# effree/EM-Spec

Hardware: AMD Instinct MI355X
Metric: reassigned spectrogram columns/sec (4096-pt, hop 256, 48 kHz) (higher is better)
Workload: dtype f32

## Files before the change

### em-spec_amd/csrc/emspec_api.cpp

```cpp
#include "emspec_engine.h"
#ifdef EMSPEC_DIAG
#pragma GCC visibility push(default)
#include "../../include/emspec_debug.h"
#pragma GCC visibility pop
#endif
#include <algorithm>
#include <cmath>
#include <cstdio>
#include <cstdlib>
#include <cstring>
#include <map>
#include <new>
#include <string>
#include <vector>

using namespace emspec;

namespace {
thread_local std::string g_create_error = "";
}

namespace emspec {
int fail(const emspec_engine* e, int code, const std::string& msg) {
    if (e) e->err = msg; else g_create_error = msg;
// ... 113 lines not shown
    p.h_tw.resize(n);
    const double pi = 3.14159265358979323846;
    for (int q = 0; q < n / 2; ++q) {
        const double a = 2.0 * pi * (double)q / (double)n;
        p.h_tw[2 * q] = (float)std::cos(a);
        p.h_tw[2 * q + 1] = (float)(-std::sin(a));
    }
    for (int q = 0; q < n / 4; ++q) {
        p.h_tw[2 * (q + n / 4)] = p.h_tw[2 * q + 1];
        p.h_tw[2 * (q + n / 4) + 1] = -p.h_tw[2 * q];
    }
    p.h_tw[2 * (n / 4)] = 0.0f;
    p.h_tw[2 * (n / 4) + 1] = -1.0f;
    const int R = e->cfg.rows;
    p.h_ebin.resize(R + 1);
    const double ratio = (double)e->cfg.fmax_hz / (double)e->cfg.fmin_hz;
    for (int r = 0; r <= R; ++r)
        p.h_ebin[r] = e->custom_edges_hz.empty()
                          ? (float)((double)e->cfg.fmin_hz * spec_pow(ratio, (double)r / (double)R) * (double)n /
                                    (double)e->cfg.sample_rate)
                          : (float)((double)e->custom_edges_hz[r] * (double)n / (double)e->cfg.sample_rate);
    for (int r = 0; r < R; ++r)
        if (!(p.h_ebin[r] < p.h_ebin[r + 1])) return fail(e, EMSPEC_ERR_INVALID_ARG, "row edges are not strictly increasing in float32 (too many rows for this range)");
    HIPCHK(e, hipMalloc(&p.d_tw, sizeof(float) * n));
    HIPCHK(e, hipMalloc(&p.d_ebin, sizeof(float) * (R + 1)));
    HIPCHK(e, hipMemcpy(p.d_tw, p.h_tw.data(), sizeof(float) * n, hipMemcpyHostToDevice));
    HIPCHK(e, hipMemcpy(p.d_ebin, p.h_ebin.data(), sizeof(float) * (R + 1), hipMemcpyHostToDevice));
    if (e->exact()) {
        std::vector<double> tw((size_t)n), eb((size_t)R + 1);
        for (int q = 0; q <= n / 8; ++q) {
            double c, sn;
            cos_sin_octant(2.0 * pi * (double)q / (double)n, &c, &sn);
            tw[2 * q] = c;
            tw[2 * q + 1] = -sn;
            if (q > 0) {
                tw[2 * (n / 4 - q)] = sn;
                tw[2 * (n / 4 - q) + 1] = -c;
            }
        }
        for (int q = 0; q < n / 4; ++q) {
            tw[2 * (q + n / 4)] = tw[2 * q + 1];
            tw[2 * (q + n / 4) + 1] = -tw[2 * q];
        }
        tw[2 * (n / 4)] = 0.0;
        tw[2 * (n / 4) + 1] = -1.0;
        for (int r = 0; r <= R; ++r)
// ... 9 lines not shown
        HIPCHK(e, hipMemcpy(p.d_tw64, tw.data(), sizeof(double) * n, hipMemcpyHostToDevice));
        HIPCHK(e, hipMemcpy(p.d_ebin64, eb.data(), sizeof(double) * (R + 1), hipMemcpyHostToDevice));
    }
    auto ins = e->plans.emplace(n, std::move(p));
    *out = &ins.first->second;
    return EMSPEC_OK;
}

int get_band_plan(emspec_engine* e, int n, int row0, int rows, Plan** out) {
    const auto key = std::make_tuple(n, row0, rows);
    auto it = e->band_plans.find(key);
    if (it != e->band_plans.end()) { *out = &it->second; return EMSPEC_OK; }
    Plan* full;
    int rc;
    if ((rc = get_plan(e, n, &full))) return rc;
    if (row0 < 0 || rows < 1 || row0 + rows > full->rows) return fail(e, EMSPEC_ERR_INVALID_ARG, "band outside the row table");
    Plan p;
    p.n = n;
    p.row0 = row0;
    p.rows = rows;
    p.d_tw = full->d_tw;
    p.d_tw64 = full->d_tw64;
    p.h_ebin.assign(full->h_ebin.begin() + row0, full->h_ebin.begin() + row0 + rows + 1);
    HIPCHK(e, hipMalloc(&p.d_ebin, sizeof(float) * (rows + 1)));
    HIPCHK(e, hipMemcpy(p.d_ebin, p.h_ebin.data(), sizeof(float) * (rows + 1), hipMemcpyHostToDevice));
    if (e->exact()) {
        HIPCHK(e, hipMalloc(&p.d_ebin64, sizeof(double) * (rows + 1)));
        HIPCHK(e, hipMemcpy(p.d_ebin64, full->d_ebin64 + row0, sizeof(double) * (rows + 1), hipMemcpyDeviceToDevice));
        HIPCHK(e, hipMemcpy(&p.h_e0, full->d_ebin64 + row0, sizeof(double), hipMemcpyDeviceToHost));
        HIPCHK(e, hipMemcpy(&p.h_eR, full->d_ebin64 + row0 + rows, sizeof(double), hipMemcpyDeviceToHost));
    }
    auto ins = e->band_plans.emplace(key, std::move(p));
    *out = &ins.first->second;
    return EMSPEC_OK;
}

PlanDev plan_dev(const emspec_engine* e, const Plan& p, int hop, int reassign) {
    PlanDev d;
    d.tw = p.d_tw;
    d.ebin = p.d_ebin;
    d.rows = p.rows;
    d.log_rows = e->custom_edges_hz.empty() ? 1 : 0;
    d.D = latency(p.n, hop, reassign);
    d.reassign = reassign ? 1 : 0;
    d.hop = hop;
    d.tscale = (float)((double)p.n / 2.0 / (double)hop);
    const double pk = (double)p.n / 4.0;
    d.pfloor_abs = (float)((double)e->cfg.power_floor * pk * pk);
    d.shared = comm_shares_device(e) ? 1 : 0;
    return d;
}

ExactPlanDev exact_plan_dev(const emspec_engine* e, const Plan& p, int hop, int reassign) {
    ExactPlanDev d;
    d.tw = p.d_tw64;
    d.ebin = p.d_ebin64;
    d.rows = p.rows;
    d.log_rows = e->custom_edges_hz.empty() ? 1 : 0;
    d.D = latency(p.n, hop, reassign);
    d.reassign = reassign ? 1 : 0;
    d.hop = hop;
    d.tscale = (double)p.n / 2.0 / (double)hop;
    const double pk = (double)p.n / 4.0;
    d.pfloor = (double)e->cfg.power_floor * pk * pk;
    int log2n = 0;
// ... 457 lines not shown


int emspec_debug_occupy(emspec_engine* e, int32_t groups, int32_t usec, void* hip_stream) {
    if (!e || groups < 1 || groups > 4096 || usec < 1 || usec > 2000000) return fail(e, EMSPEC_ERR_INVALID_ARG, "bad argument");
    HIPCHK(e, hipSetDevice(e->device));
    HIPCHK(e, launch_occupy(groups, usec, reinterpret_cast<unsigned*>(e->d_lut) + 256, (hipStream_t)hip_stream));
    return EMSPEC_OK;
}

int emspec_debug_row_lookup(emspec_engine* e, int32_t n, const float* kh, int64_t count, int32_t* out_hint,
                            int32_t* out_exact) {
    if (!e || !kh || !out_hint || !out_exact || count < 0) return fail(e, EMSPEC_ERR_INVALID_ARG, "null argument");
    int rc = check_shape(e, n, 1);
    if (rc) return rc;
    HIPCHK(e, hipSetDevice(e->device));
    Plan* p;
    if ((rc = get_plan(e, n, &p))) return rc;
    float* d_kh = nullptr; int32_t *d_a = nullptr, *d_b = nullptr;
    hipError_t r = hipMalloc(&d_kh, count * 4 + 4);
    if (r == hipSuccess) r = hipMalloc(&d_a, count * 4 + 4);
    if (r == hipSuccess) r = hipMalloc(&d_b, count * 4 + 4);
    if (r == hipSuccess) r = hipMemcpyAsync(d_kh, kh, count * 4, hipMemcpyHostToDevice, e->stream);
    if (r == hipSuccess) r = launch_row_lookup_probe(p->d_ebin, e->cfg.rows, d_kh, count, d_a, d_b, e->stream);
    if (r == hipSuccess) r = hipMemcpyAsync(out_hint, d_a, count * 4, hipMemcpyDeviceToHost, e->stream);
    if (r == hipSuccess) r = hipMemcpyAsync(out_exact, d_b, count * 4, hipMemcpyDeviceToHost, e->stream);
    if (r == hipSuccess) r = hipStreamSynchronize(e->stream);
    (void)hipFree(d_kh); (void)hipFree(d_a); (void)hipFree(d_b);
    HIPCHK(e, r);
    return EMSPEC_OK;
}

int emspec_debug_recip(emspec_engine* e, const float* d, int64_t count, float* out_short, float* out_ieee) {
    if (!e || !d || !out_short || !out_ieee || count < 0) return fail(e, EMSPEC_ERR_INVALID_ARG, "null argument");
    HIPCHK(e, hipSetDevice(e->device));
    float *d_in = nullptr, *d_a = nullptr, *d_b = nullptr;
    hipError_t r = hipMalloc(&d_in, count * 4 + 4);
    if (r == hipSuccess) r = hipMalloc(&d_a, count * 4 + 4);
    if (r == hipSuccess) r = hipMalloc(&d_b, count * 4 + 4);
    if (r == hipSuccess) r = hipMemcpyAsync(d_in, d, count * 4, hipMemcpyHostToDevice, e->stream);
    if (r == hipSuccess) r = launch_recip_probe(d_in, count, d_a, d_b, e->stream);
    if (r == hipSuccess) r = hipMemcpyAsync(out_short, d_a, count * 4, hipMemcpyDeviceToHost, e->stream);
    if (r == hipSuccess) r = hipMemcpyAsync(out_ieee, d_b, count * 4, hipMemcpyDeviceToHost, e->stream);
    if (r == hipSuccess) r = hipStreamSynchronize(e->stream);
    (void)hipFree(d_in); (void)hipFree(d_a); (void)hipFree(d_b);
    HIPCHK(e, r);
    return EMSPEC_OK;
// ... 267 lines not shown
```

### em-spec_amd/csrc/emspec_device.h

```cpp
#pragma once
#include <hip/hip_runtime.h>
#include <stdint.h>

namespace emspec {

struct PlanDev {
    const float2* tw;
    const float* ebin;
    int rows;
    int log_rows;
    int D;
    int reassign;
    int hop;
    float tscale;
    float pfloor_abs;
    int shared;
};

struct SegPlan { int seglen; int nlong; int tail; int short_last; };
__device__ __forceinline__ bool seg_of_block(const SegPlan& sp, int64_t C, int& s, int64_t& c0, int64_t& c1) {
    if (!sp.short_last) {
        s = (int)blockIdx.y;
        c0 = (int64_t)blockIdx.x * sp.seglen;
        c1 = (c0 + sp.seglen < C) ? c0 + sp.seglen : C;
// ... 150 lines not shown
        }
        int r0 = (int)((__log2f(kh) - l2e0) * rscale);
        r0 = max(0, min(r0, R - 1));
        const float lo = eb[r0], hi = eb[r0 + 1];
        r0 += (kh >= hi) ? 1 : 0;
        r0 -= (kh < lo) ? 1 : 0;
        return r0;
    }
    __device__ __forceinline__ int row_signed(float kh) const {
        if (wtop) return in_range(kh) ? row_unchecked(kh) : -1;
        return row_unchecked(kh);
    }
    __device__ __forceinline__ int row_signed_log(float kh) const {
        int r0 = (int)((__log2f(kh) - l2e0) * rscale);
        r0 = max(0, min(r0, R - 1));
        const float lo = eb[r0], hi = eb[r0 + 1];
        r0 += (kh >= hi) ? 1 : 0;
        r0 -= (kh < lo) ? 1 : 0;
        return r0;
    }
    __device__ __forceinline__ int operator()(float kh) const { return in_range(kh) ? row_unchecked(kh) : -1; }
};

constexpr float kPowerMax = 1.0e36f;
constexpr float kFastMinFloor = 1.0e-27f;

__device__ __forceinline__ float recip_normal(float d) {
    const float r = __builtin_amdgcn_rcpf(d);
    const float e = __builtin_fmaf(-d, r, 1.0f);
    const float r1 = __builtin_fmaf(e, r, r);
    const float rem = __builtin_fmaf(-d, r1, 1.0f);
    const float q1 = __builtin_fmaf(rem, r1, r1);
    const float rem2 = __builtin_fmaf(-d, q1, 1.0f);
    return __builtin_fmaf(rem2, r1, q1);
}

struct BinOut { float power; int dcol; int row; };

__device__ __forceinline__ float twice_minus(float c, float s) { return __builtin_fmaf(2.0f, c, -s); }

struct YT { float yr, yi, tr, ti; };
__device__ __forceinline__ YT split_yt(float2 z, float2 w) {
    YT o;
    o.yr = z.x + w.x; o.yi = z.y - w.y; o.tr = z.y + w.y; o.ti = w.x - z.x;
    return o;
}
// ... 33 lines not shown
    return o;
}

__device__ __forceinline__ BinOut reassign_core_fast(const PlanDev& pl, const HintLookup& lk, int k,
                                                     const YT& m, const YT& c, const YT& p) {
    const float Ar = twice_minus(c.yr, m.yr + p.yr), Ai = twice_minus(c.yi, m.yi + p.yi);
    const float Br = twice_minus(c.tr, m.tr + p.tr), Bi = twice_minus(c.ti, m.ti + p.ti);
    const float Dr = m.yr - p.yr, Di = m.yi - p.yi;
    const float den = __builtin_fmaf(Ar, Ar, Ai * Ai);
    BinOut o;
    o.power = den * 0.015625f;
    const float numT = __builtin_fmaf(Br, Ar, Bi * Ai);
    const float numF = __builtin_fmaf(Dr, Ar, Di * Ai);
    const float inv = recip_normal(den);
    const float cf = __builtin_floorf(__builtin_fmaf(numT * inv, pl.tscale, 0.5f));
    const bool ok = (o.power >= pl.pfloor_abs) && (o.power <= kPowerMax) && (__builtin_fabsf(cf) <= (float)pl.D);
    const int rr = lk.row_signed_log((float)k + numF * inv);
    o.dcol = ok ? (int)cf : 0;
    o.row = (ok && (unsigned)rr < (unsigned)lk.R) ? rr : -1;
    return o;
}
__device__ __host__ __forceinline__ bool emspec_plan_is_fast(const PlanDev& pl) {
    return pl.reassign && pl.log_rows && pl.pfloor_abs >= kFastMinFloor;
}

__device__ __forceinline__ BinOut reassign_bin(const PlanDev& pl, const float* eb, int wtop, int k,
                                               float2 zm, float2 z0, float2 zp,
                                               float2 wm, float2 w0, float2 wp) {
    ExactLookup lk{eb, pl.rows, wtop};
    return reassign_core(pl, lk, k, split_yt(zm, wm), split_yt(z0, w0), split_yt(zp, wp));
}

__device__ __forceinline__ unsigned lds_accumulate_counted(float* cell, float p, bool want) {
    unsigned* c = reinterpret_cast<unsigned*>(cell);
    bool todo = want;
    unsigned rounds = 0;
    while (__builtin_amdgcn_ballot_w64(todo) != 0ull) {
        ++rounds;
        if (todo) {
            const unsigned old = __hip_atomic_exchange(c, 0xFFFFFFFFu, __ATOMIC_RELAXED, __HIP_MEMORY_SCOPE_WORKGROUP);
            if (old != 0xFFFFFFFFu) {
                __hip_atomic_store(cell, __uint_as_float(old) + p, __ATOMIC_RELAXED, __HIP_MEMORY_SCOPE_WORKGROUP);
                todo = false;
            }
        }
    }
// ... 56 lines not shown
```

### em-spec_amd/csrc/emspec_engine.h

```cpp
#pragma once
#pragma GCC visibility push(default)
#include "../../include/emspec.h"
#pragma GCC visibility pop
#include "emspec_launch.h"

#include <functional>
#include <map>
#include <string>
#include <tuple>
#include <vector>

struct emspec_engine;
namespace emspec {
struct Plan {
    int n = 0;
    int row0 = 0, rows = 0;
    float2* d_tw = nullptr;
    float* d_ebin = nullptr;
    std::vector<float> h_tw, h_ebin;
    double2* d_tw64 = nullptr;
    double* d_ebin64 = nullptr;
    double h_e0 = 0.0, h_eR = 0.0;
};
struct LiveState {
    int S = 0, n = 0, hop = 0, reassign = -1, D = 0;
    int n_high = 0, split = 0, shift = 0, D_high = 0;
    int slots_high = 0;
    void* d_cells_high = nullptr; size_t cells_high_bytes = 0;
    int form = 0;
    int slots = 0;
    int mmax = 0;
    int64_t cap = 0;
    int ring_mask = 0;
    std::vector<int64_t> fed, emitted, seen, newbase;
    std::vector<int> pend;
    void* d_cells = nullptr; size_t cells_bytes = 0;
    float* d_sring = nullptr; size_t sring_bytes = 0;
    unsigned* d_done = nullptr; size_t done_bytes = 0;
    float* d_raw = nullptr; size_t raw_bytes = 0;
    float* d_pstate = nullptr; size_t pstate_bytes = 0;
    void* h_desc = nullptr; size_t desc_bytes = 0;
    float* h_fresh = nullptr; size_t fresh_bytes = 0;
// ... 92 lines not shown
```

### em-spec_amd/csrc/emspec_launch.h

```cpp
#pragma once
#include <hip/hip_runtime.h>
#include <stdint.h>
#include "emspec_device.h"

namespace emspec {

struct LiveStream {
    long long j0;
    long long newbase;
    int frames;
    int newcount;
    int out_at;
    int flush;
};
struct LiveSinks {
    const LiveStream* streams = nullptr;
    LiveStream uni{};
    int uniform = 0;
    const float* fresh = nullptr;
    long long fresh_stride = 0;
    float* sring = nullptr;
    int ring_mask = 0;
    unsigned* done = nullptr;
    float* out_db = nullptr;
// ... 86 lines not shown
hipError_t launch_live_post(const LiveSinks& lv, const float* raw, int raw_cols, int rows, int D, float sm, float agc, float db_top,
                            const DbMap& dm, float* pstate, int S, hipStream_t st);
int64_t wire_bound_bytes(int64_t columns, int rows);
int64_t wire_fixed_bytes(int64_t columns, int rows);
size_t wire_scratch_bytes(int64_t columns);
hipError_t launch_wire_pack(const uint8_t* index, int64_t columns, int rows, uint8_t* wire, void* scratch, hipStream_t st);
hipError_t launch_wire_unpack(const uint8_t* wire, int64_t columns, int rows, uint8_t* index, hipStream_t st);
hipError_t launch_reduce_columns(const float* db_in, const uint8_t* idx_in, int S, int64_t C, int R, int f, size_t in_stride,
                                 size_t out_stride, const uint8_t* lut, float* db_out, uint8_t* idx_out, uint8_t* rgba_out,
                                 hipStream_t st);
hipError_t launch_peaks(const float* db, int64_t columns, int R, int k, float min_db, void* peaks, hipStream_t st);
enum { kPcmS16 = 1, kPcmS24 = 2, kPcmS32 = 3, kPcmF32 = 4, kPcmMaxChannels = 8, kPcmMaxViews = 8 };
struct PcmMix { float w[kPcmMaxViews * kPcmMaxChannels]; };
hipError_t launch_pcm_decode(const void* src, int sample_type, int channels, int views, const float* mix, int sources, int64_t frames,
                             int64_t src_stride_bytes, float* out, int64_t out_stride, hipStream_t st);
bool fused_supported(int n, int hop, int rows, int reassign);
int device_cus();
#ifdef EMSPEC_DIAG
int fused_waves_per_group();
int fused_read_errflag();
hipError_t launch_row_lookup_probe(const float* ebin, int rows, const float* kh, int64_t count, int32_t* out_hint,
                                   int32_t* out_exact, hipStream_t st);
hipError_t launch_occupy(int groups, int usec, unsigned* sink, hipStream_t st);
hipError_t launch_recip_probe(const float* d, int64_t count, float* out_short, float* out_ieee, hipStream_t st);
hipError_t launch_recip64_probe(const double* d, int64_t count, double* out_short, double* out_ieee, hipStream_t st);
#endif

}
```

### em-spec_amd/csrc/fused.hip.inc

```
#include "fused_r8.hip.inc"
#include "fused_n8192.hip.inc"
#include "fused_small.hip.inc"
#include "fused_n16384.hip.inc"
#include "fused_pp.hip.inc"
#ifdef EMSPEC_DIAG
#include "diag/fused_r16.hip.inc"
#include "diag/fused_r8t.hip.inc"
#include "diag/fused_pp3.hip.inc"
#endif
namespace emspec {

#ifdef EMSPEC_DIAG
static int fused_variant() {
    static int v = -1;
    if (v < 0) {
        const char* e = getenv("EMSPEC_FUSED_VARIANT");
        v = 0;
        if (e && e[0] == 'r' && e[1] == '1') v = 1;
        if (e && e[0] == 'r' && e[1] == '8' && e[2] == 't') v = 2;
        if (e && e[0] == 'r' && e[1] == '8' && e[2] != 't') v = 3;
        if (e && e[0] == 'p' && e[1] == 'p' && e[2] == 't') v = 4;
        if (e && e[0] == 'p' && e[1] == 'p' && e[2] == '3') v = 5;
    }
    return v;
}
static int* fused_errflag() {
    static int* p[64] = {};
    int dev = 0;
    (void)hipGetDevice(&dev);
    if (!p[dev & 63]) {
        if (hipMalloc(&p[dev & 63], sizeof(int)) != hipSuccess) return nullptr;
        (void)hipMemset(p[dev & 63], 0, sizeof(int));
    }
    return p[dev & 63];
}
int fused_read_errflag() {
    int v = 0;
    int* p = fused_errflag();
    if (p) (void)hipMemcpy(&v, p, sizeof(int), hipMemcpyDeviceToHost);
    return v;
}
int fused_waves_per_group() { return fused_variant() == 1 ? 8 : 16; }
static bool diag_no_fused() {
    static int off = -1;
    if (off < 0) { const char* e = getenv("EMSPEC_NO_FUSED"); off = (e && e[0] == '1') ? 1 : 0; }
// ... 117 lines not shown
            if (pl.hop != 256) return hipErrorNotSupported;
            if (!stamps) return hipSuccess;
            return pick_bool(fast, [&](auto FA) { return go(name(std::integral_constant<int, 256>{}, std::true_type{}, FA), block, lds, stamps); });
        }
#endif
        return pick_int<256, 512, 1024>(pl.hop, [&](auto H) { return pick_bool(fast, [&](auto FA) {
            return go(name(H, std::false_type{}, FA), block, lds, nullptr);
        }); });
    };
#ifdef EMSPEC_DIAG
    if (fused_variant() == 2) {
        int* ef = fused_errflag();
        if (!ef) return hipErrorOutOfMemory;
        if (stamps) return go(fused4096_r8t_kernel<true>, block, fused_r8t_lds_bytes(pl.rows), stamps, ef);
        if (stamp_groups) return hipSuccess;
        return go(fused4096_r8t_kernel<false>, block, fused_r8t_lds_bytes(pl.rows), nullptr, ef);
    }
    if (fused_variant() == 3)
        return family(fused_r8_lds_bytes(pl.rows, pl.hop), [](auto H, auto ST, auto FA) { return fused4096_r8_kernel<H(), ST(), FA()>; });
    if (fused_variant() == 4 && fast)
        return family(fused_pp_lds_bytes(pl.rows, pl.hop), [](auto H, auto ST, auto) { return fused4096_pp3_kernel<H(), ST(), true, true>; });
    if (fused_variant() == 5)
        return family(fused_pp_lds_bytes(pl.rows, pl.hop), [](auto H, auto ST, auto FA) { return fused4096_pp3_kernel<H(), ST(), FA()>; });
    if (fused_variant() == 1) {
        if (stamps) return go(fused4096_kernel<true>, dim3(512), fused_lds_bytes(pl.rows), stamps);
        if (stamp_groups) return hipSuccess;
        return go(fused4096_kernel<false>, dim3(512), fused_lds_bytes(pl.rows), nullptr);
    }
#endif
    return family(fused_pp_lds_bytes(pl.rows, pl.hop), [](auto H, auto ST, auto FA) { return fused4096_pp_kernel<H(), ST(), FA()>; });
}

}
```

### em-spec_amd/csrc/fused_pp.hip.inc

```
namespace emspec {

#define EMSPEC_STAMP(slot)                                                        \
    if constexpr (STAMP) {                                                        \
        const unsigned long long now_ = __builtin_readcyclecounter();             \
        acc_[slot] += now_ - last_;                                               \
        last_ = now_;                                                             \
    }
template <int HOP, bool STAMP, bool FAST = false>
__global__ __launch_bounds__(1024, 4) void fused4096_pp_kernel(
    PlanDev pl, DbMap dm, const uint32_t* __restrict__ lut, const float* __restrict__ pcm, int64_t L, int64_t C,
    SegPlan sp, float* __restrict__ db, uint32_t* __restrict__ rgba, uint8_t* __restrict__ index,
    unsigned long long* __restrict__ stamps) {
    using namespace f8;
    constexpr int DMAX = Geo<HOP>::DMAX, SLOTS = Geo<HOP>::SLOTS, SH = Geo<HOP>::SH;
    unsigned long long acc_[8] = {0, 0, 0, 0, 0, 0, 0, 0};
    unsigned long long last_ = 0;
    extern __shared__ float4 smem4[];
    const int R = pl.rows, D = pl.D;
    float2* fbuf = reinterpret_cast<float2*>(smem4);
    float* ring = reinterpret_cast<float*>(fbuf + 2 * N);
    float* seb = ring + SLOTS * R;
    uint32_t* slut = reinterpret_cast<uint32_t*>(seb + R + 4);
    float2* stwB = reinterpret_cast<float2*>(slut + 256);
    float2* stwC = stwB + 7 * 64;
    unsigned* arrive = reinterpret_cast<unsigned*>(stwC + 7 * 8);

    const int tid = threadIdx.x, h = tid >> 9, t = tid & 511;
    float2* fb = fbuf + h * N;
    int s;
    int64_t c0, c1;
    if (!seg_of_block(sp, C, s, c0, c1)) return;
// ... 2 lines not shown
    const float* x0 = pcm + (size_t)s * L;

    for (int q = tid; q < SLOTS * R / 4; q += 1024) reinterpret_cast<float4*>(ring)[q] = make_float4(0.f, 0.f, 0.f, 0.f);
    for (int r = tid; r <= R; r += 1024) seb[r] = pl.ebin[r];
    if (tid < 256) slut[tid] = lut[tid];
    if (tid < 7 * 64) stwB[tid] = pl.tw[tw_index8<3>(tid >> 6, tid & 63)];
    else if (tid < 7 * 64 + 7 * 8) stwC[tid - 7 * 64] = pl.tw[tw_index8<6>((tid - 7 * 64) >> 3, (tid - 7 * 64) & 7)];
    else if (tid < 7 * 64 + 7 * 8 + 4) arrive[tid - (7 * 64 + 7 * 8)] = 0u;
    float2 twA[7];
#pragma unroll
    for (int e = 0; e < 7; ++e) twA[e] = pl.tw[tw_index8<0>(e, t)];
    float xs[8];
    {
        const int64_t j = j0 + h;
#pragma unroll
        for (int i = 0; i < 8; ++i) {
            const int64_t idx = j * HOP + t + 512 * i;
            xs[i] = idx < L ? x0[idx] : 0.0f;
        }
    }
    const float r0 = (float)(t - N / 2) * (2.0f / (float)N);
    HintLookup lk;
    lk.init(seb, pl.ebin, R, pl.log_rows);
    int posB[8], posC[8];
#pragma unroll
    for (int i = 0; i < 8; ++i) {
        posB[i] = swz(((t >> 6) << 9) + (t & 63) + (i << 6));
        posC[i] = swz(((t >> 3) << 6) + (t & 7) + (i << 3));
    }
    const int bg = ((t & 63) << 3) | (t >> 6);
    int fpos[6], mpos[6];
#pragma unroll
    for (int i = 0; i < 6; ++i) {
        fpos[i] = zpos((4 * bg - 1 + i) & (N - 1));
        mpos[i] = zpos((N - 4 * bg + 1 - i) & (N - 1));
    }
    {
        float2 v[8];
#pragma unroll
        for (int i = 0; i < 8; ++i) v[i] = make_float2(xs[i], xs[i] * (r0 + 0.25f * (float)i));
        stages8(v, TwRegsSym{twA});
        const int64_t j = j0 + h;
        if (j < C && j < jstop) {
            float2* const w0 = fb + swz(t);
            float2* const w1 = fb + (swz(t) ^ 8);
#pragma unroll
// ... 56 lines not shown
            if (spins >= (1u << 16)) { g_kernel_error = 1; break; }
            __builtin_amdgcn_s_sleep(1);
        }
        asm volatile("" ::: "memory");
        EMSPEC_STAMP(5)
        read_split6(fb, fpos, mpos, yr, yi, ur, tr);
        EMSPEC_STAMP(4)
        __syncthreads();
        EMSPEC_STAMP(6)
        {
            const int64_t jn = j + 2;
            const int64_t nx = jn * HOP + t + 512 * (8 - SH);
            float xn[SH];
#pragma unroll
            for (int q = 0; q < SH; ++q) xn[q] = (nx + 512 * q < L) ? x0[nx + 512 * q] : 0.0f;
            if (active) {
                __builtin_amdgcn_s_setprio(2);
                float* cellp[4];
                float pw[4];
                bool okv[4];
                int sbase = sk - DMAX;
                sbase += sbase < 0 ? SLOTS : 0;
                const int jrel = (int)(j - c0);
                const unsigned span = (unsigned)(c1 - c0);
                const float Df = (float)D;
                const float kf0 = (float)(4 * (((tt & 63) << 3) | (tt >> 6)));
#pragma unroll
                for (int e = 0; e < 4; ++e) {
                    const float Ar = twice_minus(yr[e + 1], yr[e] + yr[e + 2]), Ai = twice_minus(yi[e + 1], yi[e] + yi[e + 2]);
                    const float Br = twice_minus(tr[e + 1], tr[e] + tr[e + 2]), Ui = twice_minus(ur[e + 1], ur[e] + ur[e + 2]);
                    const float Dr = yr[e] - yr[e + 2], Di = yi[e] - yi[e + 2];
                    const float den = __builtin_fmaf(Ar, Ar, Ai * Ai);
                    const float Pw = den * 0.015625f;
                    bool ok = (Pw >= pl.pfloor_abs) && (Pw <= kPowerMax);
                    const float kf = kf0 + (float)e;
                    float kh = kf;
                    int d = DMAX;
                    if (FAST || pl.reassign) {
                        const float numT = __builtin_fmaf(Br, Ar, -(Ui * Ai));
                        const float numF = __builtin_fmaf(Dr, Ar, Di * Ai);
                        const float inv = FAST ? recip_normal(den) : 1.0f / den;
                        const float cf = __builtin_floorf(__builtin_fmaf(numT * inv, pl.tscale, 0.5f));
                        ok = ok && (__builtin_fabsf(cf) <= Df);
                        d = (int)cf + DMAX;
                        kh = kf + numF * inv;
                    }
                    const int rr = FAST ? lk.row_signed_log(kh) : lk.row_signed(kh);
                    ok = ok && ((unsigned)rr < (unsigned)R);
                    ok = ok && ((unsigned)(jrel + d - DMAX) < span);
                    unsigned sl = (unsigned)(sbase + d);
                    sl = min(sl, sl - (unsigned)SLOTS);
                    cellp[e] = ring + __umul24(sl, (unsigned)R) + rr;
                    pw[e] = Pw;
                    okv[e] = ok;
                }
#pragma unroll
                for (int e = 0; e < 3; ++e) {
                    const bool same = okv[e] && okv[e + 1] && (cellp[e] == cellp[e + 1]);
                    pw[e + 1] = same ? pw[e + 1] + pw[e] : pw[e + 1];
                    okv[e] = okv[e] && !same;
                }
                EMSPEC_STAMP(2)
                if constexpr (STAMP) {
                    acc_[7] += lds_accumulate_counted(cellp[0], pw[0], okv[0]);
                    acc_[7] += lds_accumulate_counted(cellp[1], pw[1], okv[1]);
                    acc_[7] += lds_accumulate_counted(cellp[2], pw[2], okv[2]);
                    acc_[7] += lds_accumulate_counted(cellp[3], pw[3], okv[3]);
                } else {
                    lds_accumulate(cellp[0], pw[0], okv[0]);
                    lds_accumulate(cellp[1], pw[1], okv[1]);
                    __builtin_amdgcn_s_setprio(1);
                    lds_accumulate(cellp[2], pw[2], okv[2]);
                    lds_accumulate(cellp[3], pw[3], okv[3]);
                }
                __builtin_amdgcn_s_setprio(0);
            }
#pragma unroll
            for (int i = 0; i < 8 - SH; ++i) xs[i] = xs[i + SH];
#pragma unroll
            for (int q = 0; q < SH; ++q) xs[8 - SH + q] = xn[q];
            float2 v[8];
#pragma unroll
            for (int i = 0; i < 8; ++i) v[i] = make_float2(xs[i], xs[i] * (r0 + 0.25f * (float)i));
// ... 29 lines not shown
```

### em-spec_amd/csrc/kernels.hip

```cpp
#include "emspec_launch.h"
#include "fused_common.hip.inc"
#include "live.hip.inc"

#include <algorithm>
#include <cstdlib>
#include <mutex>
#include <set>
#include <type_traits>
#include <utility>

#ifndef EMSPEC_BINS_UNROLL
#define EMSPEC_BINS_UNROLL 1
#endif
namespace emspec {

static hipError_t allow_max_lds(const void* fn) {
    static std::mutex mu;
    static std::set<std::pair<int, const void*>> done;
    int dev = 0;
    (void)hipGetDevice(&dev);
    std::lock_guard<std::mutex> g(mu);
    if (done.count({dev, fn})) return hipSuccess;
    const hipError_t e = hipFuncSetAttribute(fn, hipFuncAttributeMaxDynamicSharedMemorySize, 160 * 1024);
    if (e == hipSuccess) done.insert({dev, fn});
// ... 451 lines not shown
#ifdef EMSPEC_DIAG
__global__ void row_lookup_probe_kernel(const float* __restrict__ ebin, int rows, const float* __restrict__ kh,
                                        int64_t count, int32_t* __restrict__ out_hint, int32_t* __restrict__ out_exact) {
    extern __shared__ float4 smem4[];
    float* seb = reinterpret_cast<float*>(smem4);
    for (int r = threadIdx.x; r <= rows; r += blockDim.x) seb[r] = ebin[r];
    __syncthreads();
    HintLookup lk;
    lk.init(seb, ebin, rows, 1);
    int wtop = 1;
    while (wtop * 2 < rows) wtop *= 2;
    for (int64_t i = (int64_t)blockIdx.x * blockDim.x + threadIdx.x; i < count; i += (int64_t)gridDim.x * blockDim.x) {
        out_hint[i] = lk(kh[i]);
        out_exact[i] = row_lookup(seb, rows, wtop, kh[i]);
    }
}
hipError_t launch_row_lookup_probe(const float* ebin, int rows, const float* kh, int64_t count, int32_t* out_hint,
                                   int32_t* out_exact, hipStream_t st) {
    hipLaunchKernelGGL(row_lookup_probe_kernel, dim3(256), dim3(256), (size_t)(rows + 4) * 4, st, ebin, rows, kh, count,
                       out_hint, out_exact);
    return hipGetLastError();
}

__global__ void recip_probe_kernel(const float* __restrict__ d, int64_t count, float* __restrict__ out_short,
                                   float* __restrict__ out_ieee) {
    for (int64_t i = (int64_t)blockIdx.x * blockDim.x + threadIdx.x; i < count; i += (int64_t)gridDim.x * blockDim.x) {
        out_short[i] = recip_normal(d[i]);
        out_ieee[i] = 1.0f / d[i];
    }
}
hipError_t launch_recip_probe(const float* d, int64_t count, float* out_short, float* out_ieee, hipStream_t st) {
    hipLaunchKernelGGL(recip_probe_kernel, dim3(1024), dim3(256), 0, st, d, count, out_short, out_ieee);
    return hipGetLastError();
}

__global__ void occupy_kernel(long long ticks, unsigned* sink) {
    const long long t0 = wall_clock64();
    unsigned n = 0;
    for (long long it = 0; it < 400000000LL; ++it) {
        if (wall_clock64() - t0 >= ticks) break;
        __builtin_amdgcn_s_sleep(32);
        ++n;
    }
    if (threadIdx.x == 0 && blockIdx.x == 0) *sink = n;
}
hipError_t launch_occupy(int groups, int usec, unsigned* sink, hipStream_t st) {
// ... 19 lines not shown
```

### include/emspec_debug.h

```cpp
#ifndef EMSPEC_DEBUG_H
#define EMSPEC_DEBUG_H
#include "emspec.h"
#ifdef __cplusplus
extern "C" {
#endif

int emspec_debug_row_lookup(emspec_engine* e, int32_t n, const float* kh, int64_t count,
                            int32_t* out_hint, int32_t* out_exact);

int emspec_debug_recip(emspec_engine* e, const float* d, int64_t count, float* out_short, float* out_ieee);

int emspec_debug_recip64(emspec_engine* e, const double* d, int64_t count, double* out_short, double* out_ieee);

int emspec_debug_phase_cycles(emspec_engine* e, const float* pcm_dev, int32_t S, int64_t L,
                              int32_t n, int32_t hop, int32_t reassign, float* db_dev,
                              uint8_t* index_dev, uint64_t* cycles, int64_t* groups,
                              int32_t* waves);

int emspec_debug_fused_error(emspec_engine* e);

int emspec_debug_occupy(emspec_engine* e, int32_t groups, int32_t usec, void* hip_stream);

int emspec_debug_live_stamps(emspec_engine* e, uint64_t* stamps);

#ifdef __cplusplus
}
#endif
#endif
```

Baseline: 116.0 million.

## Add single-probe log row lookup and fold column bounds into reassignment clamp

Adds a HintLookup1 row lookup for log-spaced rows. It computes the row from a log2 and fma, then applies a single edge comparison, and is enabled only when a host-side error bound proves the table admits it. The per-bin column-range check is folded into clamped cf bounds, ring addressing becomes byte offsets with precomputed bases, and short-circuit booleans become bitwise ops. The goal is fewer instructions and branches in the hot accumulation path. The new lookup's correctness rests on the analytic bound, and a diagnostic pp4 kernel file plus probe API are also added.

```diff
diff --git a/em-spec_amd/csrc/diag/fused_pp4.hip.inc b/em-spec_amd/csrc/diag/fused_pp4.hip.inc
--- /dev/null
+++ b/em-spec_amd/csrc/diag/fused_pp4.hip.inc
@@ -0,0 +1,245 @@
+namespace emspec {
+
+#define EMSPEC_STAMP(slot)                                                        \
+    if constexpr (STAMP) {                                                        \
+        const unsigned long long now_ = __builtin_readcyclecounter();             \
+        acc_[slot] += now_ - last_;                                               \
+        last_ = now_;                                                             \
+    }
+template <int HOP, bool STAMP, bool FAST = false>
+__global__ __launch_bounds__(1024, 4) void fused4096_pp4_kernel(
+    PlanDev pl, DbMap dm, const uint32_t* __restrict__ lut, const float* __restrict__ pcm, int64_t L, int64_t C,
+    SegPlan sp, float* __restrict__ db, uint32_t* __restrict__ rgba, uint8_t* __restrict__ index,
+    unsigned long long* __restrict__ stamps) {
+    using namespace f8;
+    constexpr int DMAX = Geo<HOP>::DMAX, SLOTS = Geo<HOP>::SLOTS, SH = Geo<HOP>::SH;
+    unsigned long long acc_[8] = {0, 0, 0, 0, 0, 0, 0, 0};
+    unsigned long long last_ = 0;
+    extern __shared__ float4 smem4[];
+    const int R = pl.rows, D = pl.D;
+    float2* fbuf = reinterpret_cast<float2*>(smem4);
+    float* ring = reinterpret_cast<float*>(fbuf + 2 * N);
+    float* seb = ring + SLOTS * R;
+    uint32_t* slut = reinterpret_cast<uint32_t*>(seb + R + 4);
+    float2* stwB = reinterpret_cast<float2*>(slut + 256);
+    float2* stwC = stwB + 7 * 64;
+    unsigned* arrive = reinterpret_cast<unsigned*>(stwC + 7 * 8);
+
+    const int tid = threadIdx.x, h = tid >> 9, t = tid & 511;
+    float2* fb = fbuf + h * N;
+    int s;
+    int64_t c0, c1;
+    if (!seg_of_block(sp, C, s, c0, c1)) return;
+    const int64_t j0 = (c0 - D > 0 ? c0 - D : 0) & ~(int64_t)1;
+    const int64_t jstop = c1 + D;
+    const float* x0 = pcm + (size_t)s * L;
+
+    for (int q = tid; q < SLOTS * R / 4; q += 1024) reinterpret_cast<float4*>(ring)[q] = make_float4(0.f, 0.f, 0.f, 0.f);
+    for (int r = tid; r <= R; r += 1024) seb[r] = pl.ebin[r];
+    if (tid < 256) slut[tid] = lut[tid];
+    if (tid < 7 * 64) stwB[tid] = pl.tw[tw_index8<3>(tid >> 6, tid & 63)];
+    else if (tid < 7 * 64 + 7 * 8) stwC[tid - 7 * 64] = pl.tw[tw_index8<6>((tid - 7 * 64) >> 3, (tid - 7 * 64) & 7)];
+    else if (tid < 7 * 64 + 7 * 8 + 4) arrive[tid - (7 * 64 + 7 * 8)] = 0u;
+    float2 twA[7];
+#pragma unroll
+    for (int e = 0; e < 7; ++e) twA[e] = pl.tw[tw_index8<0>(e, t)];
+    float xs[8];
+    {
+        const int64_t j = j0 + h;
+#pragma unroll
+        for (int i = 0; i < 8; ++i) {
+            const int64_t idx = j * HOP + t + 512 * i;
+            xs[i] = idx < L ? x0[idx] : 0.0f;
+        }
+    }
+    const float r0 = (float)(t - N / 2) * (2.0f / (float)N);
+    HintLookup lk;
+    lk.init(seb, pl.ebin, R, pl.log_rows);
+    int posB[8], posC[8];
+#pragma unroll
+    for (int i = 0; i < 8; ++i) {
+        posB[i] = swz(((t >> 6) << 9) + (t & 63) + (i << 6));
+        posC[i] = swz(((t >> 3) << 6) + (t & 7) + (i << 3));
+    }
+    const int bg = ((t & 63) << 3) | (t >> 6);
+    int fpos[6], mpos[6];
+#pragma unroll
+    for (int i = 0; i < 6; ++i) {
+        fpos[i] = zpos((4 * bg - 1 + i) & (N - 1));
+        mpos[i] = zpos((N - 4 * bg + 1 - i) & (N - 1));
+    }
+    {
+        float2 v[8];
+#pragma unroll
+        for (int i = 0; i < 8; ++i) v[i] = make_float2(xs[i], xs[i] * (r0 + 0.25f * (float)i));
+        stages8(v, TwRegsSym{twA});
+        const int64_t j = j0 + h;
+        if (j < C && j < jstop) {
+            float2* const w0 = fb + swz(t);
+            float2* const w1 = fb + (swz(t) ^ 8);
+#pragma unroll
+            for (int i = 0; i < 8; ++i) ((i & 1) ? w1 : w0)[T * i] = v[i];
+        }
+    }
+    const int klast = (int)(c1 + 1 + D - j0);
+    const int P = (klast + 2) >> 1;
+    int sk = (int)((j0 + h) % SLOTS);
+    unsigned arrivals = 0;
+    __syncthreads();
+    unsigned long long real0_ = 0;
+    if constexpr (STAMP) { last_ = __builtin_readcyclecounter(); real0_ = __builtin_amdgcn_s_memrealtime(); }
+    if (h) __syncthreads();
+    int k = h;
+#pragma unroll 1
+    for (int p = 0; p < P; ++p, k += 2) {
+        int tt = t;
+        asm volatile("" : "+v"(tt));
+        const int64_t j = j0 + k;
+        const bool active = j < C && j < jstop;
+        float yr[6], yi[6], ur[6], tr[6];
+        if (active) {
+            float2 v[8];
+#pragma unroll
+            for (int i = 0; i < 8; ++i) v[i] = fb[posB[i]];
+            stages8(v, TwLdsSym<64>{stwB + (tt & 63)});
+#pragma unroll
+            for (int i = 0; i < 8; ++i) fb[posB[i]] = v[i];
+            wave_lds_sync();
+#pragma unroll
+            for (int i = 0; i < 8; ++i) v[i] = fb[posC[i]];
+            stages8(v, TwLdsSym<8>{stwC + (tt & 7)});
+#pragma unroll
+            for (int i = 0; i < 8; ++i) fb[posC[i]] = v[i];
+            wave_lds_sync();
+#pragma unroll
+            for (int i = 0; i < 8; ++i) v[i] = fb[swz((tt << 3) + i)];
+            fft_stages<LOG2N, 9, 3>(v, 0, pl.tw);
+#pragma unroll
+            for (int i = 0; i < 8; ++i) fb[swz((tt << 3) + i)] = v[i];
+        }
+        asm volatile("" ::: "memory");
+        if ((tt & 63) == 0) __hip_atomic_fetch_add(arrive + h, 1u, __ATOMIC_RELAXED, __HIP_MEMORY_SCOPE_WORKGROUP);
+        asm volatile("" ::: "memory");
+        arrivals += 8;
+        EMSPEC_STAMP(1)
+        {
+            const int qpc = R >> 2;
+            const int64_t col = j - 2 - D;
+            if (t < qpc && col >= c0 && col < c1) {
+                const int cell = t << 2;
+                int sl = sk - 2 - D;
+                sl += sl < 0 ? SLOTS : 0;
+                finalize_ring_quad(ring, sl, R, cell, dm, slut, ((size_t)s * C + col) * R + cell, db, rgba, index);
+            }
+        }
+        EMSPEC_STAMP(0)
+        for (unsigned spins = 0; (int)(__hip_atomic_load(arrive + h, __ATOMIC_RELAXED, __HIP_MEMORY_SCOPE_WORKGROUP) - arrivals) < 0; ++spins) {
+            if (spins >= (1u << 16)) { g_kernel_error = 1; break; }
+            __builtin_amdgcn_s_sleep(1);
+        }
+        asm volatile("" ::: "memory");
+        EMSPEC_STAMP(5)
+        read_split6(fb, fpos, mpos, yr, yi, ur, tr);
+        EMSPEC_STAMP(4)
+        __syncthreads();
+        EMSPEC_STAMP(6)
+        {
+            const int64_t jn = j + 2;
+            const int64_t nx = jn * HOP + t + 512 * (8 - SH);
+            float xn[SH];
+#pragma unroll
+            for (int q = 0; q < SH; ++q) xn[q] = (nx + 512 * q < L) ? x0[nx + 512 * q] : 0.0f;
+            if (active) {
+                __builtin_amdgcn_s_setprio(2);
+                float* cellp[4];
+                float pw[4];
+                bool okv[4];
+                int sbase = sk - DMAX;
+                sbase += sbase < 0 ? SLOTS : 0;
+                const int jrel = (int)(j - c0);
+                const unsigned span = (unsigned)(c1 - c0);
+                const float Df = (float)D;
+                const float kf0 = (float)(4 * (((tt & 63) << 3) | (tt >> 6)));
+#pragma unroll
+                for (int e = 0; e < 4; ++e) {
+                    const float Ar = twice_minus(yr[e + 1], yr[e] + yr[e + 2]), Ai = twice_minus(yi[e + 1], yi[e] + yi[e + 2]);
+                    const float Br = twice_minus(tr[e + 1], tr[e] + tr[e + 2]), Ui = twice_minus(ur[e + 1], ur[e] + ur[e + 2]);
+                    const float Dr = yr[e] - yr[e + 2], Di = yi[e] - yi[e + 2];
+                    const float den = __builtin_fmaf(Ar, Ar, Ai * Ai);
+                    const float Pw = den * 0.015625f;
+                    bool ok = (Pw >= pl.pfloor_abs) && (Pw <= kPowerMax);
+                    const float kf = kf0 + (float)e;
+                    float kh = kf;
+                    int d = DMAX;
+                    if (FAST || pl.reassign) {
+                        const float numT = __builtin_fmaf(Br, Ar, -(Ui * Ai));
+                        const float numF = __builtin_fmaf(Dr, Ar, Di * Ai);
+                        const float inv = FAST ? recip_normal(den) : 1.0f / den;
+                        const float cf = __builtin_floorf(__builtin_fmaf(numT * inv, pl.tscale, 0.5f));
+                        ok = ok && (__builtin_fabsf(cf) <= Df);
+                        d = (int)cf + DMAX;
+                        kh = kf + numF * inv;
+                    }
+                    const int rr = FAST ? lk.row_signed_log(kh) : lk.row_signed(kh);
+                    ok = ok && ((unsigned)rr < (unsigned)R);
+                    ok = ok && ((unsigned)(jrel + d - DMAX) < span);
+                    unsigned sl = (unsigned)(sbase + d);
+                    sl = min(sl, sl - (unsigned)SLOTS);
+                    cellp[e] = ring + __umul24(sl, (unsigned)R) + rr;
+                    pw[e] = Pw;
+                    okv[e] = ok;
+                }
+#pragma unroll
+                for (int e = 0; e < 3; ++e) {
+                    const bool same = okv[e] && okv[e + 1] && (cellp[e] == cellp[e + 1]);
+                    pw[e + 1] = same ? pw[e + 1] + pw[e] : pw[e + 1];
+                    okv[e] = okv[e] && !same;
+                }
+                EMSPEC_STAMP(2)
+                if constexpr (STAMP) {
+                    acc_[7] += lds_accumulate_counted(cellp[0], pw[0], okv[0]);
+                    acc_[7] += lds_accumulate_counted(cellp[1], pw[1], okv[1]);
+                    acc_[7] += lds_accumulate_counted(cellp[2], pw[2], okv[2]);
+                    acc_[7] += lds_accumulate_counted(cellp[3], pw[3], okv[3]);
+                } else {
+                    lds_accumulate(cellp[0], pw[0], okv[0]);
+                    lds_accumulate(cellp[1], pw[1], okv[1]);
+                    __builtin_amdgcn_s_setprio(1);
+                    lds_accumulate(cellp[2], pw[2], okv[2]);
+                    lds_accumulate(cellp[3], pw[3], okv[3]);
+                }
+                __builtin_amdgcn_s_setprio(0);
+            }
+#pragma unroll
+            for (int i = 0; i < 8 - SH; ++i) xs[i] = xs[i + SH];
+#pragma unroll
+            for (int q = 0; q < SH; ++q) xs[8 - SH + q] = xn[q];
+            float2 v[8];
+#pragma unroll
+            for (int i = 0; i < 8; ++i) v[i] = make_float2(xs[i], xs[i] * (r0 + 0.25f * (float)i));
+            stages8(v, TwRegsSym{twA});
+            EMSPEC_STAMP(3)
+            if (jn < C && jn < jstop) {
+                float2* const w0 = fb + swz(tt);
+                float2* const w1 = fb + (swz(tt) ^ 8);
+#pragma unroll
+                for (int i = 0; i < 8; ++i) ((i & 1) ? w1 : w0)[T * i] = v[i];
+            }
+        }
+        __syncthreads();
+        EMSPEC_STAMP(6)
+        sk += 2;
+        sk -= sk >= SLOTS ? SLOTS : 0;
+    }
+    if (!h) __syncthreads();
+    if constexpr (STAMP) {
+        if ((tid & 63) == 0) {
+            unsigned long long* o = stamps + ((size_t)(blockIdx.y * gridDim.x + blockIdx.x) * 16 + (tid >> 6)) * 8;
+            acc_[7] = (acc_[7] & 0xFFFFFFFFull) | ((__builtin_amdgcn_s_memrealtime() - real0_) << 32);
+            for (int i = 0; i < 8; ++i) o[i] = acc_[i];
+        }
+    }
+}
+#undef EMSPEC_STAMP
+
+}
diff --git a/em-spec_amd/csrc/emspec_api.cpp b/em-spec_amd/csrc/emspec_api.cpp
--- a/em-spec_amd/csrc/emspec_api.cpp
+++ b/em-spec_amd/csrc/emspec_api.cpp
@@ -1,4 +1,5 @@
 #include "emspec_engine.h"
+#include "row_hint1.h"
 #ifdef EMSPEC_DIAG
 #pragma GCC visibility push(default)
 #include "../../include/emspec_debug.h"
@@ -159,6 +160,7 @@
                           : (float)((double)e->custom_edges_hz[r] * (double)n / (double)e->cfg.sample_rate);
     for (int r = 0; r < R; ++r)
         if (!(p.h_ebin[r] < p.h_ebin[r + 1])) return fail(e, EMSPEC_ERR_INVALID_ARG, "row edges are not strictly increasing in float32 (too many rows for this range)");
+    p.row1 = row_hint1_admits(p.h_ebin.data(), R);
     HIPCHK(e, hipMalloc(&p.d_tw, sizeof(float) * n));
     HIPCHK(e, hipMalloc(&p.d_ebin, sizeof(float) * (R + 1)));
     HIPCHK(e, hipMemcpy(p.d_tw, p.h_tw.data(), sizeof(float) * n, hipMemcpyHostToDevice));
@@ -214,6 +216,7 @@
     p.d_tw = full->d_tw;
     p.d_tw64 = full->d_tw64;
     p.h_ebin.assign(full->h_ebin.begin() + row0, full->h_ebin.begin() + row0 + rows + 1);
+    p.row1 = row_hint1_admits(p.h_ebin.data(), rows);
     HIPCHK(e, hipMalloc(&p.d_ebin, sizeof(float) * (rows + 1)));
     HIPCHK(e, hipMemcpy(p.d_ebin, p.h_ebin.data(), sizeof(float) * (rows + 1), hipMemcpyHostToDevice));
     if (e->exact()) {
@@ -232,7 +235,7 @@
     d.tw = p.d_tw;
     d.ebin = p.d_ebin;
     d.rows = p.rows;
-    d.log_rows = e->custom_edges_hz.empty() ? 1 : 0;
+    d.log_rows = e->custom_edges_hz.empty() ? (p.row1 ? 3 : 1) : 0;
     d.D = latency(p.n, hop, reassign);
     d.reassign = reassign ? 1 : 0;
     d.hop = hop;
@@ -736,6 +739,29 @@
     if (r == hipSuccess) r = hipMalloc(&d_b, count * 4 + 4);
     if (r == hipSuccess) r = hipMemcpyAsync(d_kh, kh, count * 4, hipMemcpyHostToDevice, e->stream);
     if (r == hipSuccess) r = launch_row_lookup_probe(p->d_ebin, e->cfg.rows, d_kh, count, d_a, d_b, e->stream);
+    if (r == hipSuccess) r = hipMemcpyAsync(out_hint, d_a, count * 4, hipMemcpyDeviceToHost, e->stream);
+    if (r == hipSuccess) r = hipMemcpyAsync(out_exact, d_b, count * 4, hipMemcpyDeviceToHost, e->stream);
+    if (r == hipSuccess) r = hipStreamSynchronize(e->stream);
+    (void)hipFree(d_kh); (void)hipFree(d_a); (void)hipFree(d_b);
+    HIPCHK(e, r);
+    return EMSPEC_OK;
+}
+
+int emspec_debug_row_lookup1(emspec_engine* e, int32_t n, const float* kh, int64_t count, int32_t* out_hint,
+                             int32_t* out_exact, int32_t* admitted) {
+    if (!e || !kh || !out_hint || !out_exact || count < 0) return fail(e, EMSPEC_ERR_INVALID_ARG, "null argument");
+    int rc = check_shape(e, n, 1);
+    if (rc) return rc;
+    HIPCHK(e, hipSetDevice(e->device));
+    Plan* p;
+    if ((rc = get_plan(e, n, &p))) return rc;
+    if (admitted) *admitted = (e->custom_edges_hz.empty() && p->row1) ? 1 : 0;
+    float* d_kh = nullptr; int32_t *d_a = nullptr, *d_b = nullptr;
+    hipError_t r = hipMalloc(&d_kh, count * 4 + 4);
+    if (r == hipSuccess) r = hipMalloc(&d_a, count * 4 + 4);
+    if (r == hipSuccess) r = hipMalloc(&d_b, count * 4 + 4);
+    if (r == hipSuccess) r = hipMemcpyAsync(d_kh, kh, count * 4, hipMemcpyHostToDevice, e->stream);
+    if (r == hipSuccess) r = launch_row_lookup1_probe(p->d_ebin, e->cfg.rows, d_kh, count, d_a, d_b, e->stream);
     if (r == hipSuccess) r = hipMemcpyAsync(out_hint, d_a, count * 4, hipMemcpyDeviceToHost, e->stream);
     if (r == hipSuccess) r = hipMemcpyAsync(out_exact, d_b, count * 4, hipMemcpyDeviceToHost, e->stream);
     if (r == hipSuccess) r = hipStreamSynchronize(e->stream);
diff --git a/em-spec_amd/csrc/emspec_device.h b/em-spec_amd/csrc/emspec_device.h
--- a/em-spec_amd/csrc/emspec_device.h
+++ b/em-spec_amd/csrc/emspec_device.h
@@ -196,6 +196,21 @@
     __device__ __forceinline__ int operator()(float kh) const { return in_range(kh) ? row_unchecked(kh) : -1; }
 };
 
+struct HintLookup1 {
+    const float* eb; int R; float rscale, c;
+    __device__ __forceinline__ void init(const float* table, const float* gtable, int rows) {
+        eb = table; R = rows;
+        const float l2e0 = log2f(gtable[0]);
+        rscale = (float)rows / (log2f(gtable[rows]) - l2e0);
+        c = 0.5f - l2e0 * rscale;
+    }
+    __device__ __forceinline__ int row_signed_log1(float kh) const {
+        int h = (int)__builtin_fmaf(__log2f(kh), rscale, c);
+        h = max(0, min(h, R));
+        return h - ((kh < eb[h]) ? 1 : 0);
+    }
+};
+
 constexpr float kPowerMax = 1.0e36f;
 constexpr float kFastMinFloor = 1.0e-27f;
 
@@ -275,6 +290,9 @@
 }
 __device__ __host__ __forceinline__ bool emspec_plan_is_fast(const PlanDev& pl) {
     return pl.reassign && pl.log_rows && pl.pfloor_abs >= kFastMinFloor;
+}
+__device__ __host__ __forceinline__ bool emspec_plan_is_row1(const PlanDev& pl) {
+    return emspec_plan_is_fast(pl) && (pl.log_rows & 2) != 0;
 }
 
 __device__ __forceinline__ BinOut reassign_bin(const PlanDev& pl, const float* eb, int wtop, int k,
diff --git a/em-spec_amd/csrc/emspec_engine.h b/em-spec_amd/csrc/emspec_engine.h
--- a/em-spec_amd/csrc/emspec_engine.h
+++ b/em-spec_amd/csrc/emspec_engine.h
@@ -18,6 +18,7 @@
     float2* d_tw = nullptr;
     float* d_ebin = nullptr;
     std::vector<float> h_tw, h_ebin;
+    bool row1 = false;
     double2* d_tw64 = nullptr;
     double* d_ebin64 = nullptr;
     double h_e0 = 0.0, h_eR = 0.0;
diff --git a/em-spec_amd/csrc/emspec_launch.h b/em-spec_amd/csrc/emspec_launch.h
--- a/em-spec_amd/csrc/emspec_launch.h
+++ b/em-spec_amd/csrc/emspec_launch.h
@@ -132,6 +132,8 @@
 hipError_t launch_row_lookup_probe(const float* ebin, int rows, const float* kh, int64_t count, int32_t* out_hint,
                                    int32_t* out_exact, hipStream_t st);
 hipError_t launch_occupy(int groups, int usec, unsigned* sink, hipStream_t st);
+hipError_t launch_row_lookup1_probe(const float* ebin, int rows, const float* kh, int64_t count, int32_t* out_hint,
+                                    int32_t* out_exact, hipStream_t st);
 hipError_t launch_recip_probe(const float* d, int64_t count, float* out_short, float* out_ieee, hipStream_t st);
 hipError_t launch_recip64_probe(const double* d, int64_t count, double* out_short, double* out_ieee, hipStream_t st);
 #endif
diff --git a/em-spec_amd/csrc/fused.hip.inc b/em-spec_amd/csrc/fused.hip.inc
--- a/em-spec_amd/csrc/fused.hip.inc
+++ b/em-spec_amd/csrc/fused.hip.inc
@@ -7,6 +7,7 @@
 #include "diag/fused_r16.hip.inc"
 #include "diag/fused_r8t.hip.inc"
 #include "diag/fused_pp3.hip.inc"
+#include "diag/fused_pp4.hip.inc"
 #endif
 namespace emspec {
 
@@ -21,6 +22,8 @@
         if (e && e[0] == 'r' && e[1] == '8' && e[2] != 't') v = 3;
         if (e && e[0] == 'p' && e[1] == 'p' && e[2] == 't') v = 4;
         if (e && e[0] == 'p' && e[1] == 'p' && e[2] == '3') v = 5;
+        if (e && e[0] == 'p' && e[1] == 'p' && e[2] == '4') v = 6;
+        if (e && e[0] == 'p' && e[1] == 'p' && e[2] == 's') v = 7;
     }
     return v;
 }
@@ -184,12 +187,16 @@
         return family(fused_pp_lds_bytes(pl.rows, pl.hop), [](auto H, auto ST, auto) { return fused4096_pp3_kernel<H(), ST(), true, true>; });
     if (fused_variant() == 5)
         return family(fused_pp_lds_bytes(pl.rows, pl.hop), [](auto H, auto ST, auto FA) { return fused4096_pp3_kernel<H(), ST(), FA()>; });
+    if (fused_variant() == 6)
+        return family(fused_pp_lds_bytes(pl.rows, pl.hop), [](auto H, auto ST, auto FA) { return fused4096_pp4_kernel<H(), ST(), FA()>; });
     if (fused_variant() == 1) {
         if (stamps) return go(fused4096_kernel<true>, dim3(512), fused_lds_bytes(pl.rows), stamps);
         if (stamp_groups) return hipSuccess;
         return go(fused4096_kernel<false>, dim3(512), fused_lds_bytes(pl.rows), nullptr);
     }
 #endif
+    if (emspec_plan_is_row1(pl) && fused_variant() != 7)
+        return family(fused_pp_lds_bytes(pl.rows, pl.hop), [](auto H, auto ST, auto) { return fused4096_pp_kernel<H(), ST(), true, true>; });
     return family(fused_pp_lds_bytes(pl.rows, pl.hop), [](auto H, auto ST, auto FA) { return fused4096_pp_kernel<H(), ST(), FA()>; });
 }
 
diff --git a/em-spec_amd/csrc/fused_pp.hip.inc b/em-spec_amd/csrc/fused_pp.hip.inc
--- a/em-spec_amd/csrc/fused_pp.hip.inc
+++ b/em-spec_amd/csrc/fused_pp.hip.inc
@@ -6,7 +6,7 @@
         acc_[slot] += now_ - last_;                                               \
         last_ = now_;                                                             \
     }
-template <int HOP, bool STAMP, bool FAST = false>
+template <int HOP, bool STAMP, bool FAST = false, bool ROW1 = false>
 __global__ __launch_bounds__(1024, 4) void fused4096_pp_kernel(
     PlanDev pl, DbMap dm, const uint32_t* __restrict__ lut, const float* __restrict__ pcm, int64_t L, int64_t C,
     SegPlan sp, float* __restrict__ db, uint32_t* __restrict__ rgba, uint8_t* __restrict__ index,
@@ -55,6 +55,8 @@
     const float r0 = (float)(t - N / 2) * (2.0f / (float)N);
     HintLookup lk;
     lk.init(seb, pl.ebin, R, pl.log_rows);
+    HintLookup1 lk1;
+    lk1.init(seb, pl.ebin, R);
     int posB[8], posC[8];
 #pragma unroll
     for (int i = 0; i < 8; ++i) {
@@ -157,8 +159,11 @@
                 int sbase = sk - DMAX;
                 sbase += sbase < 0 ? SLOTS : 0;
                 const int jrel = (int)(j - c0);
-                const unsigned span = (unsigned)(c1 - c0);
-                const float Df = (float)D;
+                const int span = (int)(c1 - c0);
+                const float cflo = (float)max(-D, -jrel), cfhi = (float)min(D, span - 1 - jrel);
+                const int colb = R << 2;
+                const int sboff = __mul24(sbase + DMAX, colb);
+                const unsigned ringb = (unsigned)(SLOTS * colb);
                 const float kf0 = (float)(4 * (((tt & 63) << 3) | (tt >> 6)));
 #pragma unroll
                 for (int e = 0; e < 4; ++e) {
@@ -167,33 +172,34 @@
                     const float Dr = yr[e] - yr[e + 2], Di = yi[e] - yi[e + 2];
                     const float den = __builtin_fmaf(Ar, Ar, Ai * Ai);
                     const float Pw = den * 0.015625f;
-                    bool ok = (Pw >= pl.pfloor_abs) && (Pw <= kPowerMax);
+                    bool ok = (Pw >= pl.pfloor_abs) & (Pw <= kPowerMax);
                     const float kf = kf0 + (float)e;
                     float kh = kf;
-                    int d = DMAX;
+                    int icf = 0;
                     if (FAST || pl.reassign) {
                         const float numT = __builtin_fmaf(Br, Ar, -(Ui * Ai));
                         const float numF = __builtin_fmaf(Dr, Ar, Di * Ai);
                         const float inv = FAST ? recip_normal(den) : 1.0f / den;
                         const float cf = __builtin_floorf(__builtin_fmaf(numT * inv, pl.tscale, 0.5f));
-                        ok = ok && (__builtin_fabsf(cf) <= Df);
-                        d = (int)cf + DMAX;
+                        ok = ok & (cf >= cflo) & (cf <= cfhi);
+                        icf = (int)cf;
                         kh = kf + numF * inv;
+                    } else {
+                        ok = ok & (0.0f >= cflo) & (0.0f <= cfhi);
                     }
-                    const int rr = FAST ? lk.row_signed_log(kh) : lk.row_signed(kh);
-                    ok = ok && ((unsigned)rr < (unsigned)R);
-                    ok = ok && ((unsigned)(jrel + d - DMAX) < span);
-                    unsigned sl = (unsigned)(sbase + d);
-                    sl = min(sl, sl - (unsigned)SLOTS);
-                    cellp[e] = ring + __umul24(sl, (unsigned)R) + rr;
+                    const int rr = ROW1 ? lk1.row_signed_log1(kh) : (FAST ? lk.row_signed_log(kh) : lk.row_signed(kh));
+                    ok = ok & ((unsigned)rr < (unsigned)R);
+                    unsigned off = (unsigned)(__mul24(icf, colb) + sboff);
+                    off = min(off, off - ringb);
+                    cellp[e] = reinterpret_cast<float*>(reinterpret_cast<char*>(ring) + off) + rr;
                     pw[e] = Pw;
                     okv[e] = ok;
                 }
 #pragma unroll
                 for (int e = 0; e < 3; ++e) {
-                    const bool same = okv[e] && okv[e + 1] && (cellp[e] == cellp[e + 1]);
+                    const bool same = okv[e] & okv[e + 1] & (cellp[e] == cellp[e + 1]);
                     pw[e + 1] = same ? pw[e + 1] + pw[e] : pw[e + 1];
-                    okv[e] = okv[e] && !same;
+                    okv[e] = okv[e] & !same;
                 }
                 EMSPEC_STAMP(2)
                 if constexpr (STAMP) {
diff --git a/em-spec_amd/csrc/kernels.hip b/em-spec_amd/csrc/kernels.hip
--- a/em-spec_amd/csrc/kernels.hip
+++ b/em-spec_amd/csrc/kernels.hip
@@ -497,6 +497,28 @@
     return hipGetLastError();
 }
 
+__global__ void row_lookup1_probe_kernel(const float* __restrict__ ebin, int rows, const float* __restrict__ kh,
+                                         int64_t count, int32_t* __restrict__ out_hint, int32_t* __restrict__ out_exact) {
+    extern __shared__ float4 smem4[];
+    float* seb = reinterpret_cast<float*>(smem4);
+    for (int r = threadIdx.x; r <= rows; r += blockDim.x) seb[r] = ebin[r];
+    __syncthreads();
+    HintLookup1 lk;
+    lk.init(seb, ebin, rows);
+    int wtop = 1;
+    while (wtop * 2 < rows) wtop *= 2;
+    for (int64_t i = (int64_t)blockIdx.x * blockDim.x + threadIdx.x; i < count; i += (int64_t)gridDim.x * blockDim.x) {
+        out_hint[i] = lk.row_signed_log1(kh[i]);
+        out_exact[i] = kh[i] >= seb[rows] ? rows : row_lookup(seb, rows, wtop, kh[i]);
+    }
+}
+hipError_t launch_row_lookup1_probe(const float* ebin, int rows, const float* kh, int64_t count, int32_t* out_hint,
+                                    int32_t* out_exact, hipStream_t st) {
+    hipLaunchKernelGGL(row_lookup1_probe_kernel, dim3(256), dim3(256), (size_t)(rows + 4) * 4, st, ebin, rows, kh, count,
+                       out_hint, out_exact);
+    return hipGetLastError();
+}
+
 __global__ void recip_probe_kernel(const float* __restrict__ d, int64_t count, float* __restrict__ out_short,
                                    float* __restrict__ out_ieee) {
     for (int64_t i = (int64_t)blockIdx.x * blockDim.x + threadIdx.x; i < count; i += (int64_t)gridDim.x * blockDim.x) {
diff --git a/em-spec_amd/csrc/row_hint1.h b/em-spec_amd/csrc/row_hint1.h
--- /dev/null
+++ b/em-spec_amd/csrc/row_hint1.h
@@ -0,0 +1,33 @@
+#pragma once
+#include <cmath>
+
+namespace emspec {
+
+struct RowHint1Bound {
+    double dev;
+    double arith;
+};
+
+inline RowHint1Bound row_hint1_bound(const float* eb, int R) {
+    const double L0 = std::log2((double)eb[0]), LR = std::log2((double)eb[R]);
+    const double span = LR - L0, rs = (double)R / span;
+    RowHint1Bound b{0.0, 0.0};
+    for (int r = 0; r <= R; ++r) {
+        const double d = std::fabs((std::log2((double)eb[r]) - L0) * rs - (double)r);
+        if (d > b.dev) b.dev = d;
+    }
+    const double lmax = std::fmax(std::fabs(L0), std::fabs(LR)) + 1.0 / rs;
+    const double rho = 2.0 * lmax * 0x1p-22 / span + 0x1p-23;
+    b.arith = lmax * 0x1p-23 * rs + lmax * rs * rho + std::fabs(L0) * rs * (rho + 0x1p-22 + 0x1p-24) +
+              (std::fabs(L0) * rs + 0.5) * 0x1p-24 + ((double)R + 2.0) * 0x1p-24;
+    return b;
+}
+
+constexpr double kRowHint1Room = 0.25;
+inline bool row_hint1_admits(const float* eb, int R) {
+    if (R < 1 || !(eb[0] > 0.0f) || !(eb[R] > eb[0]) || !std::isfinite(eb[R])) return false;
+    const RowHint1Bound b = row_hint1_bound(eb, R);
+    return b.dev + b.arith <= kRowHint1Room;
+}
+
+}
diff --git a/include/emspec_debug.h b/include/emspec_debug.h
--- a/include/emspec_debug.h
+++ b/include/emspec_debug.h
@@ -7,6 +7,9 @@
 
 int emspec_debug_row_lookup(emspec_engine* e, int32_t n, const float* kh, int64_t count,
                             int32_t* out_hint, int32_t* out_exact);
+
+int emspec_debug_row_lookup1(emspec_engine* e, int32_t n, const float* kh, int64_t count,
+                             int32_t* out_hint, int32_t* out_exact, int32_t* admitted);
 
 int emspec_debug_recip(emspec_engine* e, const float* d, int64_t count, float* out_short, float* out_ieee);
 
```

Result: no change. 116.1 million (median of 2 runs) (+0.0%).
